# calmiLovesAI/ComputerVision.pytorch

Measured on AMD Instinct MI355X. Metric: images/sec 640x640 YOLOv8-n train step, higher is better.
Workload: dtype f16; 1 GPU; YOLOv8-n train step (fwd + v8 loss + bwd + Adam), batch 32/GPU, 640x640, nc=80, random init; global_batch=32, parallelism=dp1, launch=eager, exchange=none (1 rank), gpu_max_hw_queues=4

## Files before the change

computervision.pytorch_amd/csrc/stem.hip:

```cpp
#include "stem.h"

#include "bn_common.h"

namespace {
using namespace cvx_bn;

constexpr int KT = 27;

struct PixelId {
  int b, oy, ox;
};
__device__ __forceinline__ PixelId pixel_of(const StemParams& p, long long m) {
  const unsigned mu = (unsigned)m;
  const unsigned t = mu / (unsigned)p.OW;
  const int ox = (int)(mu - t * (unsigned)p.OW);
  const int b = (int)(t / (unsigned)p.OH);
  const int oy = (int)(t - (unsigned)b * (unsigned)p.OH);
  return PixelId{b, oy, ox};
}

__device__ __forceinline__ void load_window(const StemParams& p, const PixelId& id, float (&x)[KT]) {
  const long long plane = (long long)p.H * p.W;
  const float* img = p.img + (long long)id.b * 3 * plane;
#pragma unroll
  for (int kh = 0; kh < 3; ++kh) {
    const int iy = 2 * id.oy - 1 + kh;
    const bool rok = iy >= 0;
    const int iyc = rok ? iy : 0;
#pragma unroll
    for (int ci = 0; ci < 3; ++ci) {
      const float* row = img + ci * plane + (long long)iyc * p.W + 2 * id.ox;
      const float2 c = *reinterpret_cast<const float2*>(row);
      const float l = id.ox > 0 ? row[-1] : 0.f;
      x[(kh * 3 + 0) * 3 + ci] = rok ? l : 0.f;
      x[(kh * 3 + 1) * 3 + ci] = rok ? c.x : 0.f;
      x[(kh * 3 + 2) * 3 + ci] = rok ? c.y : 0.f;
    }
  }
}

__device__ __forceinline__ void stage_weights(const StemParams& p, float* sW) {
  for (int i = threadIdx.x; i < KT * p.Cout; i += blockDim.x) {
    const int co = i / KT, k = i - co * KT;
    sW[k * p.Cout + co] = p.w[i];
  }
}

__device__ __forceinline__ void conv16(const float (&x)[KT], const float* sW, int Cout, int g, float (&acc)[16]) {
#pragma unroll
  for (int c = 0; c < 16; ++c) acc[c] = 0.f;
#pragma unroll
  for (int k = 0; k < KT; ++k) {
    const f4* w4 = reinterpret_cast<const f4*>(sW + k * Cout + g * 16);
#pragma unroll
    for (int q = 0; q < 4; ++q) {
      const f4 w = w4[q];
#pragma unroll
      for (int r = 0; r < 4; ++r) acc[q * 4 + r] = fmaf(x[k], w[r], acc[q * 4 + r]);
    }
  }
}

template <int NG>
__global__ __launch_bounds__(256) void stem_stats_kernel(const StemParams p, long long M, long long* stats) {
  extern __shared__ __attribute__((aligned(16))) float smem[];
  float* sW = smem;
  float* sred = smem + KT * p.Cout;
  stage_weights(p, sW);
  __syncthreads();
  float s1[NG][16], s2[NG][16];
#pragma unroll
  for (int g = 0; g < NG; ++g)
#pragma unroll
    for (int c = 0; c < 16; ++c) s1[g][c] = s2[g][c] = 0.f;
  for (long long m = (long long)blockIdx.x * 256 + threadIdx.x; m < M; m += (long long)gridDim.x * 256) {
    asm volatile("" ::: "memory");
    const PixelId id = pixel_of(p, m);
    float x[KT];
    load_window(p, id, x);
#pragma unroll
    for (int g = 0; g < NG; ++g) {
      float acc[16];
      conv16(x, sW, p.Cout, g, acc);
#pragma unroll
      for (int c = 0; c < 16; ++c) {
        s1[g][c] += acc[c];
        s2[g][c] = fmaf(acc[c], acc[c], s2[g][c]);
      }
    }
  }
  const int wave = threadIdx.x >> 6, lane = threadIdx.x & 63;
#pragma unroll
  for (int g = 0; g < NG; ++g)
#pragma unroll
    for (int c = 0; c < 16; ++c) {
      const float a = cvx_wave_sum64(s1[g][c]), b = cvx_wave_sum64(s2[g][c]);
      if (lane == 0) {
        sred[(wave * 2 + 0) * p.Cout + g * 16 + c] = a;
        sred[(wave * 2 + 1) * p.Cout + g * 16 + c] = b;
      }
    }
  __syncthreads();
  for (int t = threadIdx.x; t < 2 * p.Cout; t += 256) {
    const int which = t / p.Cout, c = t - which * p.Cout;
    const float v = (sred[(0 * 2 + which) * p.Cout + c] + sred[(1 * 2 + which) * p.Cout + c]) +
                    (sred[(2 * 2 + which) * p.Cout + c] + sred[(3 * 2 + which) * p.Cout + c]);
    cvx_fix_atomic_add(stats, ((long long)(blockIdx.x % cvx_stat_replicas(p.Cout)) * p.Cout + c) * 2 + which, v);
  }
}

template <int NG, bool TRAIN>
__global__ __launch_bounds__(256) void stem_apply_kernel(const StemParams p, long long M, BnTrainArgs a, const float* scale,
                                                         const float* shift, ViewDesc out, half_t* xhat) {
  extern __shared__ __attribute__((aligned(16))) long long ws[];
  float* sA = reinterpret_cast<float*>(reinterpret_cast<char*>(ws) + (TRAIN ? fold_ws_bytes(p.Cout) : 0));
  float* sB = sA + p.Cout;
  float* sG = sB + p.Cout;
  float* sBe = sG + p.Cout;
  float* sW = sBe + p.Cout;
  if (TRAIN) {
    fold_replicas(a.stats, p.Cout, ws);
    for (int c = threadIdx.x; c < p.Cout; c += 256) {
      double var;
      const BnMoments mo = moments_of(ws, p.Cout, c, M, a.eps, &var);
      sA[c] = mo.mean;
      sB[c] = mo.invstd;
      sG[c] = a.gamma[c];
      sBe[c] = a.beta[c];
      if (blockIdx.x == 0) {
        const double cnt = (double)M;
        const double mu = reinterpret_cast<const double*>(ws)[c] / cnt;
        a.mean[c] = mo.mean;
        a.invstd[c] = mo.invstd;
        const double unbiased = cnt > 1.0 ? var * cnt / (cnt - 1.0) : var;
        a.rmean[c] = (float)((1.0 - a.momentum) * (double)a.rmean[c] + a.momentum * mu);
        a.rvar[c] = (float)((1.0 - a.momentum) * (double)a.rvar[c] + a.momentum * unbiased);
      }
    }
  } else {
    for (int c = threadIdx.x; c < p.Cout; c += 256) {
      sA[c] = scale[c];
      sB[c] = shift[c];
    }
  }
  stage_weights(p, sW);
  __syncthreads();
  const int ohw = p.OH * p.OW;
  for (long long m = (long long)blockIdx.x * 256 + threadIdx.x; m < M; m += (long long)gridDim.x * 256) {
    asm volatile("" ::: "memory");
    const PixelId id = pixel_of(p, m);
    float x[KT];
    load_window(p, id, x);
    half_t* o = out.p + (long long)id.b * out.bstride + ((long long)id.oy * p.OW + id.ox) * out.ld;
#pragma unroll
    for (int g = 0; g < NG; ++g) {
      float acc[16];
      conv16(x, sW, p.Cout, g, acc);
      h8 av[2], xv[2];
#pragma unroll
      for (int c = 0; c < 16; ++c) {
        const int ch = g * 16 + c;
        float z;
        if (TRAIN) {
          const float xh = (acc[c] - sA[ch]) * sB[ch];
          xv[c >> 3][c & 7] = (half_t)xh;
          z = fmaf(xh, sG[ch], sBe[ch]);
        } else {
          z = fmaf(acc[c], sA[ch], sB[ch]);
        }
        av[c >> 3][c & 7] = (half_t)cvx_silu(z);
      }
      *reinterpret_cast<h8*>(o + g * 16) = av[0];
      *reinterpret_cast<h8*>(o + g * 16 + 8) = av[1];
      if (TRAIN && xhat) {
        half_t* xo = xhat + m * p.Cout + g * 16;
        *reinterpret_cast<h8*>(xo) = xv[0];
        *reinterpret_cast<h8*>(xo + 8) = xv[1];
      }
    }
  }
  (void)ohw;
}

__global__ __launch_bounds__(256) void stem_wgrad_kernel(const StemParams p, long long M, const half_t* dy, float* slabs) {
  const int wave = threadIdx.x >> 6, lane = threadIdx.x & 63;
  const int co0 = blockIdx.y * 16 + wave * 4;
  float acc[4][KT];
#pragma unroll
  for (int c = 0; c < 4; ++c)
#pragma unroll
    for (int k = 0; k < KT; ++k) acc[c][k] = 0.f;
  constexpr int WG_UNR = 3;
  const long long stride = (long long)gridDim.x * 64;
  for (long long m0 = (long long)blockIdx.x * 64 + lane; m0 < M; m0 += stride * WG_UNR) {
    asm volatile("" ::: "memory");
    float x[WG_UNR][KT];
    h4 g[WG_UNR];
#pragma unroll
    for (int u = 0; u < WG_UNR; ++u) {
      const long long m = m0 + u * stride;
      const bool ok = m < M;
      const long long mm = ok ? m : m0;
      load_window(p, pixel_of(p, mm), x[u]);
      g[u] = *reinterpret_cast<const h4*>(dy + mm * p.Cout + co0);
      if (!ok) g[u] = h4{(half_t)0, (half_t)0, (half_t)0, (half_t)0};
    }
#pragma unroll
    for (int u = 0; u < WG_UNR; ++u)
#pragma unroll
      for (int c = 0; c < 4; ++c) {
        const float gc = (float)g[u][c];
#pragma unroll
        for (int k = 0; k < KT; ++k) acc[c][k] = fmaf(gc, x[u][k], acc[c][k]);
      }
  }
  float* slab = slabs + (long long)blockIdx.x * p.Cout * 144;
#pragma unroll
  for (int c = 0; c < 4; ++c)
#pragma unroll
    for (int k = 0; k < KT; ++k) {
      const float v = cvx_wave_sum64(acc[c][k]);
      if (lane == 0) slab[(co0 + c) * 144 + (k / 3) * 16 + (k % 3)] = v;
    }
}

__global__ __launch_bounds__(256) void stem_bwd_kernel(const StemParams p, long long M, const half_t* xhat, ViewDesc gout, BnCoef k,
                                                       const long long* part, float inv_scale, float* dgamma, float* dbeta, float* slabs,
                                                       int tiles_x, int tiles_y, int total_tiles) {
  constexpr int TH = 8, TW = 32, WR = 2 * TH + 1, WE = TW + 1, WO = TW;
  constexpr int ROWP = WE + WO + 1;
  extern __shared__ __attribute__((aligned(16))) long long ws[];
  float* sG = reinterpret_cast<float*>(reinterpret_cast<char*>(ws) + fold_ws_bytes(p.Cout));
  float* sB = sG + p.Cout;
  float* sK1 = sB + p.Cout;
  float* sK2 = sK1 + p.Cout;
  float* sGi = sK2 + p.Cout;
  float* sX = sGi + p.Cout;
  fold_replicas(part, p.Cout, ws);
  {
    const double* s0 = reinterpret_cast<const double*>(ws);
    const double* s1 = s0 + p.Cout;
    const double cnt = (double)M;
    for (int c = threadIdx.x; c < p.Cout; c += 256) {
      const float g = k.gamma[c];
      sG[c] = g;
      sB[c] = k.beta[c];
      sK1[c] = (float)(s0[c] / cnt);
      sK2[c] = (float)(s1[c] / cnt);
      sGi[c] = g * k.invstd[c];
      if (blockIdx.x == 0 && blockIdx.y == 0) {
        dgamma[c] += (float)(s1[c] * inv_scale);
        dbeta[c] += (float)(s0[c] * inv_scale);
      }
    }
  }
  __syncthreads();
  const int wave = threadIdx.x >> 6, lane = threadIdx.x & 63;
  const int co0 = blockIdx.y * 16 + wave * 4;
  float ga[4], be[4], k1[4], k2[4], gi[4];
#pragma unroll
  for (int c = 0; c < 4; ++c) {
    ga[c] = sG[co0 + c];
    be[c] = sB[co0 + c];
    k1[c] = sK1[co0 + c];
    k2[c] = sK2[co0 + c];
    gi[c] = sGi[co0 + c];
  }
  float acc[4][KT];
#pragma unroll
  for (int c = 0; c < 4; ++c)
#pragma unroll
    for (int kk = 0; kk < KT; ++kk) acc[c][kk] = 0.f;
  const long long plane = (long long)p.H * p.W;
  const int lx = lane & 31, ly = lane >> 5;
  for (int tile = blockIdx.x; tile < total_tiles; tile += gridDim.x) {
    const int tx = tile % tiles_x;
    const int t2 = tile / tiles_x;
    const int ty = t2 % tiles_y;
    const int b = t2 / tiles_y;
    const int oy0 = ty * TH, ox0 = tx * TW;
    auto load_group = [&](int q, h4& xq, h4& gq, bool& okq) {
      const int oy = oy0 + q * 2 + ly, ox = ox0 + lx;
      okq = oy < p.OH && ox < p.OW;
      const long long pix = okq ? (long long)oy * p.OW + ox : 0;
      xq = *reinterpret_cast<const h4*>(xhat + ((long long)b * p.OH * p.OW + pix) * p.Cout + co0);
      gq = *reinterpret_cast<const h4*>(gout.p + (long long)b * gout.bstride + pix * gout.ld + co0);
    };
    h4 xn, gn;
    bool okn;
    load_group(0, xn, gn, okn);
    const float* img = p.img + (long long)b * 3 * plane;
    __syncthreads();
    {
      constexpr int NE = 3 * WR * (WE + WO), NST = (NE + 255) / 256;
      float v[NST];
      int dst[NST];
#pragma unroll
      for (int it = 0; it < NST; ++it) {
        const int e = it * 256 + threadIdx.x;
        const int j = e % (WE + WO);
        const int t3 = e / (WE + WO);
        const int r = t3 % WR, ci = t3 / WR;
        const int iy = 2 * oy0 - 1 + r, ix = 2 * ox0 - 1 + j;
        const bool in = e < NE && iy >= 0 && iy < p.H && ix >= 0 && ix < p.W;
        v[it] = in ? img[ci * plane + (long long)iy * p.W + ix] : 0.f;
        dst[it] = e < NE ? (ci * WR + r) * ROWP + ((j & 1) ? WE + (j >> 1) : (j >> 1)) : -1;
      }
#pragma unroll
      for (int it = 0; it < NST; ++it)
        if (dst[it] >= 0) sX[dst[it]] = v[it];
    }
    __syncthreads();
#pragma unroll 1
    for (int q = 0; q < 4; ++q) {
      const h4 xq = xn, gq = gn;
      const bool okq = okn;
      if (q < 3) load_group(q + 1, xn, gn, okn);
      float dyc[4];
#pragma unroll
      for (int c = 0; c < 4; ++c) {
        const float xv = (float)xq[c];
        const float dz = (float)gq[c] * cvx_silu_grad(xv * ga[c] + be[c]);
        dyc[c] = okq ? (float)(half_t)(gi[c] * (dz - k1[c] - xv * k2[c])) : 0.f;
      }
      const float* rowq = sX + (2 * (q * 2 + ly)) * ROWP;
#pragma unroll
      for (int kh = 0; kh < 3; ++kh)
#pragma unroll
        for (int ci = 0; ci < 3; ++ci) {
          const float* row = rowq + (ci * WR + kh) * ROWP;
          const float x0 = row[lx], x1 = row[WE + lx], x2 = row[lx + 1];
#pragma unroll
          for (int c = 0; c < 4; ++c) {
            acc[c][(kh * 3 + 0) * 3 + ci] = fmaf(dyc[c], x0, acc[c][(kh * 3 + 0) * 3 + ci]);
            acc[c][(kh * 3 + 1) * 3 + ci] = fmaf(dyc[c], x1, acc[c][(kh * 3 + 1) * 3 + ci]);
            acc[c][(kh * 3 + 2) * 3 + ci] = fmaf(dyc[c], x2, acc[c][(kh * 3 + 2) * 3 + ci]);
          }
        }
    }
  }
  float* slab = slabs + (long long)blockIdx.x * p.Cout * 144;
#pragma unroll
  for (int c = 0; c < 4; ++c)
#pragma unroll
    for (int kk = 0; kk < KT; ++kk) {
      const float v = cvx_wave_sum64(acc[c][kk]);
      if (lane == 0) slab[(co0 + c) * 144 + (kk / 3) * 16 + (kk % 3)] = v;
    }
}

constexpr int SM_TH = 8, SM_TW = 32, SM_WR = 2 * SM_TH + 1, SM_P = 72, SM_PL = SM_WR * SM_P + 16;
constexpr int SM_WIN_CHUNKS = 16 * 64;
constexpr int SM_STAGE_BYTES = SM_WIN_CHUNKS * 16 + 2 * SM_TH * SM_TW * 32;
static_assert(3 * SM_PL / 4 <= SM_WIN_CHUNKS, "window chunks");

typedef __attribute__((address_space(3))) void* stem_lds_ptr;

constexpr int SM_PART = 16 * 32 * 2 + 32 + 16 + 16;

template <bool ONEPASS, bool RECOMP = false>
__global__ __launch_bounds__(256) void stem_bwd_mfma_kernel(const StemParams p, long long M, const half_t* xhat, ViewDesc gout, BnCoef k,
                                                            const long long* part, float inv_scale, float* dgamma, float* dbeta, float* slabs,
                                                            int tiles_x, int tiles_y, int total_tiles) {
#if defined(__HIP_DEVICE_COMPILE__)
  extern __shared__ __attribute__((aligned(16))) long long ws[];
  float* sG = reinterpret_cast<float*>(reinterpret_cast<char*>(ws) + fold_ws_bytes(p.Cout));
  float* sB = sG + p.Cout;
  float* sK1 = sB + p.Cout;
  float* sK2 = sK1 + p.Cout;
  float* sGi = sK2 + p.Cout;
  unsigned char* stage0 = reinterpret_cast<unsigned char*>(reinterpret_cast<uintptr_t>(sGi + p.Cout + 3) & ~(uintptr_t)15);
  const int wave = __builtin_amdgcn_readfirstlane(threadIdx.x >> 6), lane = threadIdx.x & 63;
  const int g = lane >> 4, m = lane & 15;
  const int co0 = blockIdx.y * 16;
  const long long plane = (long long)p.H * p.W;

  const __amdgpu_buffer_rsrc_t rs_img = __builtin_amdgcn_make_buffer_rsrc(const_cast<float*>(p.img), (short)0, (int)(unsigned)((long long)p.B * 3 * plane * 4), 0x00020000);
  const __amdgpu_buffer_rsrc_t rs_xh = __builtin_amdgcn_make_buffer_rsrc(const_cast<half_t*>(xhat), (short)0, (int)(unsigned)(M * p.Cout * 2), 0x00020000);
  const __amdgpu_buffer_rsrc_t rs_g = __builtin_amdgcn_make_buffer_rsrc(gout.p, (short)0, (int)(unsigned)((long long)p.B * gout.bstride * 2), 0x00020000);

  int w_rel[4], w_r[4], w_j[4];
#pragma unroll
  for (int j = 0; j < 4; ++j) {
    const int chunk = (4 * j + wave) * 64 + lane;
    const int ci = chunk / (SM_PL / 4), rem = chunk - ci * (SM_PL / 4);
    const int r = rem / (SM_P / 4), cj = rem - r * (SM_P / 4);
    const bool used = ci < 3 && r < SM_WR && cj < 17;
    w_r[j] = used ? r : -100000;
    w_j[j] = cj;
    w_rel[j] = (int)((ci * (long long)p.H + (r - 1)) * p.W + (4 * cj - 4)) * 4;
  }
  const int t_px = lane >> 1, t_half = lane & 1;

  auto issue = [&](int tile, unsigned char* st) {
    const int tx = tile % tiles_x;
    const int t2 = tile / tiles_x;
    const int ty = t2 % tiles_y;
    const int b = t2 / tiles_y;
    const int oy0 = ty * SM_TH, ox0 = tx * SM_TW;
    const unsigned base = (unsigned)((((long long)b * 3 * p.H + 2 * oy0) * p.W + 2 * ox0) * 4);
#pragma unroll
    for (int j = 0; j < 4; ++j) {
      const int iy = 2 * oy0 - 1 + w_r[j], ix = 2 * ox0 - 4 + 4 * w_j[j];
      const bool ok = iy >= 0 && iy < p.H && ix >= 0 && ix < p.W;
      const unsigned vo = ok ? base + (unsigned)w_rel[j] : 0xffffffffu;
      __builtin_amdgcn_raw_ptr_buffer_load_lds(rs_img, (stem_lds_ptr)(st + (4 * j + wave) * 1024), 16, vo, 0, 0, 0);
    }
    unsigned char* sx = st + SM_WIN_CHUNKS * 16;
    unsigned char* sg = sx + (RECOMP ? 0 : SM_TH * SM_TW * 32);
#pragma unroll
    for (int j = 0; j < 2; ++j) {
      const int row = 2 * wave + j;
      const int oy = oy0 + row, ox = ox0 + t_px;
      const bool ok = oy < p.OH && ox < p.OW;
      const long long pix = (long long)oy * p.OW + ox;
      const unsigned vx = ok ? (unsigned)((((long long)b * p.OH * p.OW + pix) * p.Cout + co0) * 2 + t_half * 16) : 0xffffffffu;
      const unsigned vg = ok ? (unsigned)(((long long)b * gout.bstride + pix * gout.ld + co0) * 2 + t_half * 16) : 0xffffffffu;
      if constexpr (!RECOMP) __builtin_amdgcn_raw_ptr_buffer_load_lds(rs_xh, (stem_lds_ptr)(sx + row * 1024), 16, vx, 0, 0, 0);
      __builtin_amdgcn_raw_ptr_buffer_load_lds(rs_g, (stem_lds_ptr)(sg + row * 1024), 16, vg, 0, 0, 0);
    }
  };

  int tile = blockIdx.x;
  if (tile < total_tiles) issue(tile, stage0);

  float k1 = 0.f, k2 = 0.f, gi = 0.f;
  if constexpr (!ONEPASS) {
    fold_replicas(part, p.Cout, ws);
    const double* s0 = reinterpret_cast<const double*>(ws);
    const double* s1 = s0 + p.Cout;
    const double cnt = (double)M;
    for (int c = threadIdx.x; c < p.Cout; c += 256) {
      const float gm = k.gamma[c];
      sK1[c] = (float)(s0[c] / cnt);
      sK2[c] = (float)(s1[c] / cnt);
      sGi[c] = gm * k.invstd[c];
      if (blockIdx.x == 0 && blockIdx.y == 0) {
        dgamma[c] += (float)(s1[c] * inv_scale);
        dbeta[c] += (float)(s0[c] * inv_scale);
      }
    }
    __syncthreads();
    k1 = sK1[co0 + m];
    k2 = sK2[co0 + m];
    gi = sGi[co0 + m];
  }
  const float ga = k.gamma[co0 + m], be = k.beta[co0 + m];

  int boff[2];
#pragma unroll
  for (int t = 0; t < 2; ++t) {
    const int kk = min(16 * t + m, KT - 1);
    const int ci = kk % 3, kw = (kk / 3) % 3, kh = kk / 9;
    boff[t] = (ci * SM_PL + (4 * wave + kh) * SM_P + kw + 3 + 2 * g) * 4;
  }
  const int aoff = (2 * wave * SM_TW + g) * 32 + m * 2;
  int toff7[7], boffr[2];
  float wreg[7];
  float mean_c = 0.f, invstd_c = 0.f;
  if constexpr (RECOMP) {
#pragma unroll
    for (int t = 0; t < 7; ++t) {
      const int kq = 4 * t + g, kk = min(kq, KT - 1);
      const int ci = kk % 3, kw = (kk / 3) % 3, kh = kk / 9;
      toff7[t] = (ci * SM_PL + (4 * wave + kh) * SM_P + kw + 3 + 2 * m) * 4;
      wreg[t] = kq < KT ? p.w[(long long)(co0 + m) * KT + kq] : 0.f;
    }
#pragma unroll
    for (int t = 0; t < 2; ++t) boffr[t] = boff[t] + (2 * (4 * g) - 2 * g) * 4;
    mean_c = k.mean[co0 + m];
    invstd_c = k.invstd[co0 + m];
  }
  const int aoffr = (2 * wave * SM_TW + 4 * g) * 32 + m * 2;

  f4 acc0 = {0.f, 0.f, 0.f, 0.f}, acc1 = {0.f, 0.f, 0.f, 0.f};
  f4 acx0 = {0.f, 0.f, 0.f, 0.f}, acx1 = {0.f, 0.f, 0.f, 0.f};
  float sdz = 0.f, sdzx = 0.f, sb0 = 0.f, sb1 = 0.f;
  int cur = 0;
  for (; tile < total_tiles; tile += gridDim.x) {
    constexpr int STAGE = SM_STAGE_BYTES - (RECOMP ? SM_TH * SM_TW * 32 : 0);
    unsigned char* st = stage0 + cur * STAGE;
    asm volatile("s_waitcnt vmcnt(0)" ::: "memory");
    asm volatile("" ::: "memory");
    __builtin_amdgcn_s_barrier();
    asm volatile("" ::: "memory");
    if (tile + (int)gridDim.x < total_tiles) issue(tile + gridDim.x, stage0 + (cur ^ 1) * STAGE);
    const int tx = tile % tiles_x, ty = (tile / tiles_x) % tiles_y;
    const int oy0 = ty * SM_TH + 2 * wave, ox0 = tx * SM_TW + g;
    const unsigned char* sw = st;
    const unsigned char* sx = st + SM_WIN_CHUNKS * 16 + aoff;
    const unsigned char* sg = sx + SM_TH * SM_TW * 32;
    if constexpr (ONEPASS && RECOMP) {
      const unsigned char* sgr = st + SM_WIN_CHUNKS * 16 + aoffr;
      const int oxb = tx * SM_TW + 4 * g;
#pragma unroll
      for (int q = 0; q < 4; ++q) {
        const int row = q >> 1, cb = (q & 1) * 16;
        f4 y = {0.f, 0.f, 0.f, 0.f};
#pragma unroll
        for (int t = 0; t < 7; ++t) {
          const float a = *reinterpret_cast<const float*>(sw + toff7[t] + (row * 2 * SM_P + 2 * cb) * 4);
          y = __builtin_amdgcn_mfma_f32_16x16x4f32(a, wreg[t], y, 0, 0, 0);
        }
        typedef _Float16 hv4 __attribute__((ext_vector_type(4)));
        hv4 dz4, xv4, b04, b14;
#pragma unroll
        for (int i = 0; i < 4; ++i) {
          const bool ok = oy0 + row < p.OH && oxb + cb + i < p.OW;
          const half_t xh = (half_t)((y[i] - mean_c) * invstd_c);
          const float xv = ok ? (float)xh : 0.f;
          const float gv = (float)*reinterpret_cast<const half_t*>(sgr + (row * SM_TW + cb + i) * 32);
          const half_t b0 = (half_t)*reinterpret_cast<const float*>(sw + boffr[0] + (row * 2 * SM_P + 2 * (cb + i)) * 4);
          const half_t b1 = (half_t)*reinterpret_cast<const float*>(sw + boffr[1] + (row * 2 * SM_P + 2 * (cb + i)) * 4);
          const half_t dzh = (half_t)(gv * cvx_silu_grad(xv * ga + be));
          const float dz = (float)dzh;
          dz4[i] = dzh;
          xv4[i] = (half_t)xv;
          b04[i] = b0;
          b14[i] = b1;
          sdz += dz;
          sdzx = fmaf(dz, xv, sdzx);
          sb0 += ok ? (float)b0 : 0.f;
          sb1 += ok ? (float)b1 : 0.f;
        }
        acc0 = __builtin_amdgcn_mfma_f32_16x16x16f16(dz4, b04, acc0, 0, 0, 0);
        acc1 = __builtin_amdgcn_mfma_f32_16x16x16f16(dz4, b14, acc1, 0, 0, 0);
        acx0 = __builtin_amdgcn_mfma_f32_16x16x16f16(xv4, b04, acx0, 0, 0, 0);
        acx1 = __builtin_amdgcn_mfma_f32_16x16x16f16(xv4, b14, acx1, 0, 0, 0);
      }
    } else {
#pragma unroll
    for (int s = 0; s < 16; ++s) {
      const int row = s >> 3, c4 = (s & 7) * 4;
      const float xv = (float)*reinterpret_cast<const half_t*>(sx + s * 128);
      const float gv = (float)*reinterpret_cast<const half_t*>(sg + s * 128);
      const float b0 = *reinterpret_cast<const float*>(sw + boff[0] + (row * 2 * SM_P + 2 * c4) * 4);
      const float b1 = *reinterpret_cast<const float*>(sw + boff[1] + (row * 2 * SM_P + 2 * c4) * 4);
      const bool ok = oy0 + row < p.OH && ox0 + c4 < p.OW;
      const float dz = gv * cvx_silu_grad(xv * ga + be);
      if constexpr (ONEPASS) {
        acc0 = __builtin_amdgcn_mfma_f32_16x16x4f32(dz, b0, acc0, 0, 0, 0);
        acc1 = __builtin_amdgcn_mfma_f32_16x16x4f32(dz, b1, acc1, 0, 0, 0);
        acx0 = __builtin_amdgcn_mfma_f32_16x16x4f32(xv, b0, acx0, 0, 0, 0);
        acx1 = __builtin_amdgcn_mfma_f32_16x16x4f32(xv, b1, acx1, 0, 0, 0);
        sdz += dz;
        sdzx = fmaf(dz, xv, sdzx);
        sb0 += ok ? b0 : 0.f;
        sb1 += ok ? b1 : 0.f;
      } else {
        const float dy = ok ? (float)(half_t)(gi * (dz - k1 - xv * k2)) : 0.f;
        acc0 = __builtin_amdgcn_mfma_f32_16x16x4f32(dy, b0, acc0, 0, 0, 0);
        acc1 = __builtin_amdgcn_mfma_f32_16x16x4f32(dy, b1, acc1, 0, 0, 0);
      }
    }
    }
    cur ^= 1;
  }
  if constexpr (ONEPASS) {
    __syncthreads();
    float* red = reinterpret_cast<float*>(stage0);
    float* mine = red + wave * SM_PART;
    sdz += __shfl_xor(sdz, 16);
    sdz += __shfl_xor(sdz, 32);
    sdzx += __shfl_xor(sdzx, 16);
    sdzx += __shfl_xor(sdzx, 32);
    sb0 += __shfl_xor(sb0, 16);
    sb0 += __shfl_xor(sb0, 32);
    sb1 += __shfl_xor(sb1, 16);
    sb1 += __shfl_xor(sb1, 32);
#pragma unroll
    for (int i = 0; i < 4; ++i) {
      mine[(4 * g + i) * 32 + m] = acc0[i];
      mine[(4 * g + i) * 32 + 16 + m] = acc1[i];
      mine[512 + (4 * g + i) * 32 + m] = acx0[i];
      mine[512 + (4 * g + i) * 32 + 16 + m] = acx1[i];
    }
    if (g == 0) {
      mine[1024 + m] = sb0;
      mine[1024 + 16 + m] = sb1;
      mine[1056 + m] = sdz;
      mine[1072 + m] = sdzx;
    }
    __syncthreads();
    float* out = slabs + (long long)blockIdx.x * p.Cout * 144 + blockIdx.y * (16 * 144);
    for (int e = threadIdx.x; e < SM_PART; e += 256) out[e] = ((red[e] + red[e + SM_PART]) + red[e + 2 * SM_PART]) + red[e + 3 * SM_PART];
    if (blockIdx.x == 0 && threadIdx.x == 0) reinterpret_cast<unsigned*>(out)[2 * SM_PART + 64] = 0u;
    return;
  }
  __syncthreads();
  float* red = reinterpret_cast<float*>(stage0);
#pragma unroll
  for (int i = 0; i < 4; ++i) {
    red[((wave * 2 + 0) * 4 + i) * 64 + lane] = acc0[i];
    red[((wave * 2 + 1) * 4 + i) * 64 + lane] = acc1[i];
  }
  __syncthreads();
  float* slab = slabs + (long long)blockIdx.x * p.Cout * 144;
  for (int e = threadIdx.x; e < 512; e += 256) {
    const int l = e & 63, i = (e >> 6) & 3, t = e >> 8;
    const int kk = 16 * t + (l & 15), co = 4 * (l >> 4) + i;
    if (kk < KT) {
      const int q = (t * 4 + i) * 64 + l;
      const float v = ((red[q] + red[q + 512]) + red[q + 1024]) + red[q + 1536];
      slab[(co0 + co) * 144 + (kk / 3) * 16 + (kk % 3)] = v;
    }
  }
#endif
}

constexpr int SM_FOLD_BLOCKS = SM_PART / 16;
__global__ __launch_bounds__(256) void stem_onepass_fold_kernel(float* slabs, int nsplit, int Cout, long long M, const float* gamma, const float* invstd,
                                                                float inv_scale, float* dw, float* dgamma, float* dbeta) {
  __shared__ double sd[256];
  __shared__ double col[SM_PART];
  __shared__ bool last;
  const int slice = blockIdx.y;
  const long long stride = (long long)Cout * 144;
  float* base = slabs + slice * (16 * 144);
  const int c = threadIdx.x & 15, r = threadIdx.x >> 4;
  const int column = blockIdx.x * 16 + c;
  double a = 0.0;
  int sp = r;
  for (; sp + 7 * 16 < nsplit; sp += 8 * 16) {
    float v[8];
#pragma unroll
    for (int u = 0; u < 8; ++u) v[u] = base[(long long)(sp + 16 * u) * stride + column];
#pragma unroll
    for (int u = 0; u < 8; ++u) a += (double)v[u];
  }
  for (; sp < nsplit; sp += 16) a += (double)base[(long long)sp * stride + column];
  sd[threadIdx.x] = a;
  __syncthreads();
  for (int off = 128; off >= 16; off >>= 1) {
    if ((int)threadIdx.x < off) sd[threadIdx.x] += sd[threadIdx.x + off];
    __syncthreads();
  }
  auto colsum_at = [&](int q) -> double* { return reinterpret_cast<double*>(base + (long long)(q / 544) * stride + SM_PART) + (q % 544); };
  if (threadIdx.x < 16) __hip_atomic_store(colsum_at(column), sd[threadIdx.x], __ATOMIC_RELAXED, __HIP_MEMORY_SCOPE_AGENT);
  __syncthreads();
  if (threadIdx.x == 0) {
    __threadfence();
    unsigned* ctr = reinterpret_cast<unsigned*>(base) + 2 * SM_PART + 64;
    last = atomicAdd(ctr, 1u) == gridDim.x - 1;
    if (last) __threadfence();
  }
  __syncthreads();
  if (!last) return;
  for (int q = threadIdx.x; q < SM_PART; q += 256) col[q] = __hip_atomic_load(colsum_at(q), __ATOMIC_RELAXED, __HIP_MEMORY_SCOPE_AGENT);
  __syncthreads();
  const double cnt = (double)M;
  for (int e = threadIdx.x; e < 16 * KT; e += 256) {
    const int co = e / KT, kk = e - co * KT;
    const double k1 = col[1056 + co] / cnt, k2 = col[1072 + co] / cnt;
    const double g = (double)gamma[slice * 16 + co] * (double)invstd[slice * 16 + co];
    const double v = g * (col[co * 32 + kk] - k1 * col[1024 + kk] - k2 * col[512 + co * 32 + kk]);
    dw[(long long)(slice * 16 + co) * KT + kk] += (float)(v * inv_scale);
  }
  if (threadIdx.x < 16) {
    dgamma[slice * 16 + threadIdx.x] += (float)(col[1072 + threadIdx.x] * inv_scale);
    dbeta[slice * 16 + threadIdx.x] += (float)(col[1056 + threadIdx.x] * inv_scale);
  }
}

__global__ __launch_bounds__(256) void stem_slab_fold_kernel(const float* slabs, int nsplit, int Cout, float inv_scale, float* dw) {
  const int e = blockIdx.x * 256 + threadIdx.x;
  if (e >= Cout * KT) return;
  const int co = e / KT, kk = e - co * KT;
  const float* s = slabs + (long long)co * 144 + (kk / 3) * 16 + (kk % 3);
  float a = 0.f;
  for (int sp = 0; sp < nsplit; ++sp) a += s[(long long)sp * Cout * 144];
  dw[e] += a * inv_scale;
}

int stem_grid(long long M, int per_block) {
  long long blocks = (M + per_block - 1) / per_block;
  const long long cap = 256 * 8;
  return (int)(blocks < cap ? blocks : cap);
}

int check(const StemParams& p) {
  CVX_CHECK(p.img && p.w, "stem: null pointers");
  CVX_CHECK(p.H % 2 == 0 && p.W % 2 == 0 && p.OH == p.H / 2 && p.OW == p.W / 2, "stem: even input sizes, output = input / 2");
  CVX_CHECK(p.Cout % 16 == 0 && p.Cout >= 16 && p.Cout <= 80, "stem: 16..80 output channels in multiples of 16");
  CVX_CHECK((long long)p.B * p.OH * p.OW < (1LL << 31), "stem: too many output pixels");
  CVX_CHECK(((uintptr_t)p.img % 8) == 0, "stem: images must be 8-byte aligned");
  return 0;
}

}

int cvx_stem_stats(const StemParams& p, long long* stats, hipStream_t st) {
  CVX_TRY(check(p));
  const long long M = (long long)p.B * p.OH * p.OW;
  const int lds = (KT + 8) * p.Cout * 4;
  const dim3 grid(stem_grid(M, 256));
  switch (p.Cout / 16) {
    case 1: hipLaunchKernelGGL(stem_stats_kernel<1>, grid, dim3(256), lds, st, p, M, stats); break;
    case 2: hipLaunchKernelGGL(stem_stats_kernel<2>, grid, dim3(256), lds, st, p, M, stats); break;
    case 3: hipLaunchKernelGGL(stem_stats_kernel<3>, grid, dim3(256), lds, st, p, M, stats); break;
    case 4: hipLaunchKernelGGL(stem_stats_kernel<4>, grid, dim3(256), lds, st, p, M, stats); break;
    default: hipLaunchKernelGGL(stem_stats_kernel<5>, grid, dim3(256), lds, st, p, M, stats); break;
  }
  CVX_HIP(hipGetLastError());
  return 0;
}

template <bool TRAIN>
static int launch_apply(const StemParams& p, const BnTrainArgs& a, const float* scale, const float* shift, const ViewDesc& out,
                        half_t* xhat, hipStream_t st) {
  const long long M = (long long)p.B * p.OH * p.OW;
  const int lds = (TRAIN ? fold_ws_bytes(p.Cout) : 0) + (4 + KT) * p.Cout * 4;
  const dim3 grid(stem_grid(M, 256));
  switch (p.Cout / 16) {
    case 1: hipLaunchKernelGGL((stem_apply_kernel<1, TRAIN>), grid, dim3(256), lds, st, p, M, a, scale, shift, out, xhat); break;
    case 2: hipLaunchKernelGGL((stem_apply_kernel<2, TRAIN>), grid, dim3(256), lds, st, p, M, a, scale, shift, out, xhat); break;
    case 3: hipLaunchKernelGGL((stem_apply_kernel<3, TRAIN>), grid, dim3(256), lds, st, p, M, a, scale, shift, out, xhat); break;
    case 4: hipLaunchKernelGGL((stem_apply_kernel<4, TRAIN>), grid, dim3(256), lds, st, p, M, a, scale, shift, out, xhat); break;
    default: hipLaunchKernelGGL((stem_apply_kernel<5, TRAIN>), grid, dim3(256), lds, st, p, M, a, scale, shift, out, xhat); break;
  }
  CVX_HIP(hipGetLastError());
  return 0;
}

int cvx_stem_apply_train(const StemParams& p, const BnTrainArgs& a, const ViewDesc& out, half_t* xhat, hipStream_t st) {
  CVX_TRY(check(p));
  CVX_CHECK(out.p && ((uintptr_t)out.p % 16) == 0 && out.ld % 8 == 0, "stem: output view");
  return launch_apply<true>(p, a, nullptr, nullptr, out, xhat, st);
}

int cvx_stem_apply_eval(const StemParams& p, const float* scale, const float* shift, const ViewDesc& out, hipStream_t st) {
  CVX_TRY(check(p));
  CVX_CHECK(out.p && scale && shift && ((uintptr_t)out.p % 16) == 0 && out.ld % 8 == 0, "stem: output view");
  BnTrainArgs none{};
  return launch_apply<false>(p, none, scale, shift, out, nullptr, st);
}

int cvx_stem_wgrad_splits(long long M) {
  static const int cap = cvx_tune_int("CVX_STEM_SPLITS", 512);
  return stem_grid(M, 64 * 16) < cap ? stem_grid(M, 64 * 16) : cap;
}

int cvx_stem_wgrad(const StemParams& p, const half_t* dy, float* slabs, int nsplit, hipStream_t st) {
  CVX_TRY(check(p));
  const long long M = (long long)p.B * p.OH * p.OW;
  CVX_CHECK(dy && slabs && nsplit >= 1 && nsplit == cvx_stem_wgrad_splits(M), "stem wgrad: split count must come from cvx_stem_wgrad_splits");
  hipLaunchKernelGGL(stem_wgrad_kernel, dim3(nsplit, p.Cout / 16), dim3(256), 0, st, p, M, dy, slabs);
  CVX_HIP(hipGetLastError());
  return 0;
}

int cvx_stem_backward(const StemParams& p, const half_t* xhat, const ViewDesc& gout, const BnCoef& k, const long long* part, float inv_scale,
                      float* dgamma, float* dbeta, float* slabs, int nsplit, hipStream_t st) {
  CVX_TRY(check(p));
  const long long M = (long long)p.B * p.OH * p.OW;
  CVX_CHECK(xhat && gout.p && part && dgamma && dbeta && slabs && nsplit == cvx_stem_wgrad_splits(M), "stem backward: bad arguments");
  CVX_CHECK(gout.ld % 4 == 0 && ((uintptr_t)gout.p % 8) == 0, "stem backward: gradient view alignment");
  const int tiles_x = (p.OW + 31) / 32, tiles_y = (p.OH + 7) / 8;
  static const bool mfma_on = cvx_tune_int("CVX_STEM_BWD_MFMA", 1) != 0;
  const bool mfma_ok = mfma_on && p.W % 4 == 0 && ((uintptr_t)p.img % 16) == 0 && ((uintptr_t)xhat % 16) == 0 && ((uintptr_t)gout.p % 16) == 0 &&
                       gout.ld % 8 == 0 && gout.bstride % 8 == 0 && (long long)p.B * 3 * p.H * p.W * 4 < (1LL << 32) && M * p.Cout * 2 < (1LL << 32) &&
                       (long long)p.B * gout.bstride * 2 < (1LL << 32);
  if (mfma_ok) {
    const int lds_m = fold_ws_bytes(p.Cout) + 5 * p.Cout * 4 + 32 + 2 * SM_STAGE_BYTES;
    hipLaunchKernelGGL(stem_bwd_mfma_kernel<false>, dim3(nsplit, p.Cout / 16), dim3(256), lds_m, st, p, M, xhat, gout, k, part, inv_scale, dgamma, dbeta,
                       slabs, tiles_x, tiles_y, tiles_x * tiles_y * p.B);
    CVX_HIP(hipGetLastError());
    return 0;
  }
  const int lds = fold_ws_bytes(p.Cout) + 5 * p.Cout * 4 + 3 * 17 * 66 * 4;
  hipLaunchKernelGGL(stem_bwd_kernel, dim3(nsplit, p.Cout / 16), dim3(256), lds, st, p, M, xhat, gout, k, part, inv_scale, dgamma, dbeta, slabs,
                     tiles_x, tiles_y, tiles_x * tiles_y * p.B);
  CVX_HIP(hipGetLastError());
  return 0;
}

static bool stem_dma_ok(const StemParams& p, const half_t* xhat, const ViewDesc& gout, long long M) {
  return p.W % 4 == 0 && ((uintptr_t)p.img % 16) == 0 && ((uintptr_t)xhat % 16) == 0 && ((uintptr_t)gout.p % 16) == 0 && gout.ld % 8 == 0 &&
         gout.bstride % 8 == 0 && (long long)p.B * 3 * p.H * p.W * 4 < (1LL << 32) && M * p.Cout * 2 < (1LL << 32) &&
         (long long)p.B * gout.bstride * 2 < (1LL << 32);
}
bool cvx_stem_keeps_xhat(const StemParams& p, const ViewDesc& gout, int nsplit) {
  static const bool recomp = cvx_tune_int("CVX_STEM_RECOMP", 1) != 0;
  return !(recomp && cvx_stem_backward_onepass_ok(p, reinterpret_cast<const half_t*>((uintptr_t)16), gout, nsplit));
}
bool cvx_stem_backward_onepass_ok(const StemParams& p, const half_t* xhat, const ViewDesc& gout, int nsplit) {
  static const bool on = cvx_tune_int("CVX_STEM_ONEPASS", 1) != 0;
  const long long M = (long long)p.B * p.OH * p.OW;
  return on && nsplit >= 2 && p.Cout % 16 == 0 && stem_dma_ok(p, xhat, gout, M);
}
int cvx_stem_backward_fold(const StemParams& p, const half_t* xhat, const ViewDesc& gout, const BnCoef& k, const long long* part, float inv_scale,
                           float* dgamma, float* dbeta, float* dw, float* slabs, int nsplit, hipStream_t st) {
  CVX_TRY(check(p));
  const long long M = (long long)p.B * p.OH * p.OW;
  CVX_CHECK(xhat && gout.p && dgamma && dbeta && dw && slabs && nsplit == cvx_stem_wgrad_splits(M), "stem backward: bad arguments");
  if (cvx_stem_backward_onepass_ok(p, xhat, gout, nsplit)) {
    const int tiles_x = (p.OW + 31) / 32, tiles_y = (p.OH + 7) / 8;
    const int lds_m = fold_ws_bytes(p.Cout) + 5 * p.Cout * 4 + 32 + 2 * SM_STAGE_BYTES;
    if (k.mean && !cvx_stem_keeps_xhat(p, gout, nsplit)) {
      hipLaunchKernelGGL((stem_bwd_mfma_kernel<true, true>), dim3(nsplit, p.Cout / 16), dim3(256), lds_m - 2 * SM_TH * SM_TW * 32, st, p, M, xhat, gout, k, (const long long*)nullptr,
                         inv_scale, dgamma, dbeta, slabs, tiles_x, tiles_y, tiles_x * tiles_y * p.B);
    } else
    hipLaunchKernelGGL(stem_bwd_mfma_kernel<true>, dim3(nsplit, p.Cout / 16), dim3(256), lds_m, st, p, M, xhat, gout, k, (const long long*)nullptr, inv_scale,
                       dgamma, dbeta, slabs, tiles_x, tiles_y, tiles_x * tiles_y * p.B);
    hipLaunchKernelGGL(stem_onepass_fold_kernel, dim3(SM_FOLD_BLOCKS, p.Cout / 16), dim3(256), 0, st, slabs, nsplit, p.Cout, M, k.gamma, k.invstd, inv_scale,
                       dw, dgamma, dbeta);
    CVX_HIP(hipGetLastError());
    return 0;
  }
  CVX_CHECK(part, "stem backward: the two-pass path needs the sums of bn_bwd_reduce");
  CVX_TRY(cvx_stem_backward(p, xhat, gout, k, part, inv_scale, dgamma, dbeta, slabs, nsplit, st));
  hipLaunchKernelGGL(stem_slab_fold_kernel, dim3((p.Cout * KT + 255) / 256), dim3(256), 0, st, slabs, nsplit, p.Cout, inv_scale, dw);
  CVX_HIP(hipGetLastError());
  return 0;
}
```

Measured before the change: 5676 images/sec.

## Add quad-tiled stem stats kernel that shares input windows across 2x2 outputs

```diff
diff --git a/computervision.pytorch_amd/csrc/stem.hip b/computervision.pytorch_amd/csrc/stem.hip
--- a/computervision.pytorch_amd/csrc/stem.hip
+++ b/computervision.pytorch_amd/csrc/stem.hip
@@ -180,6 +180,152 @@
     }
   }
   (void)ohw;
+}
+
+struct QuadId {
+  int b, rp, cp;
+};
+__device__ __forceinline__ QuadId quad_of(int q, int RP, int CP) {
+  const unsigned t = (unsigned)q / (unsigned)CP;
+  const int cp = (int)((unsigned)q - t * (unsigned)CP);
+  const int b = (int)(t / (unsigned)RP);
+  return QuadId{b, (int)(t - (unsigned)b * (unsigned)RP), cp};
+}
+constexpr int QW = 5 * 3;
+
+__device__ __forceinline__ void load_quad(const StemParams& p, const QuadId& id, int lane, f4 (&c)[QW], float (&l)[QW]) {
+  const long long plane = (long long)p.H * p.W;
+  const float* img = p.img + (long long)id.b * 3 * plane + 4 * id.cp;
+  const float* row[QW];
+#pragma unroll
+  for (int r = 0; r < 5; ++r) {
+    const int iy = 4 * id.rp - 1 + r;
+    const int iyc = iy < 0 ? 0 : (iy < p.H ? iy : p.H - 1);
+#pragma unroll
+    for (int ci = 0; ci < 3; ++ci) {
+      row[r * 3 + ci] = img + ci * plane + (long long)iyc * p.W;
+      c[r * 3 + ci] = *reinterpret_cast<const f4*>(row[r * 3 + ci]);
+      l[r * 3 + ci] = 0.f;
+    }
+  }
+  if (lane == 0 && id.cp > 0) {
+#pragma unroll
+    for (int i = 0; i < QW; ++i) l[i] = row[i][-1];
+  }
+}
+__device__ __forceinline__ void build_window(const QuadId& id, int lane, bool bot, const f4 (&c)[QW], const float (&l)[QW], float (&x)[5 * QW]) {
+  const bool from_lane = lane != 0 && id.cp > 0;
+#pragma unroll
+  for (int r = 0; r < 5; ++r) {
+    const bool rok = r == 0 ? id.rp > 0 : (r >= 3 ? bot : true);
+#pragma unroll
+    for (int ci = 0; ci < 3; ++ci) {
+      const f4 v = c[r * 3 + ci];
+      const float prev = cvx_dpp_mov<0x138>(v[3]);
+      x[(r * 5 + 0) * 3 + ci] = rok ? (from_lane ? prev : l[r * 3 + ci]) : 0.f;
+#pragma unroll
+      for (int j = 0; j < 4; ++j) x[(r * 5 + 1 + j) * 3 + ci] = rok ? v[j] : 0.f;
+    }
+  }
+}
+__device__ __forceinline__ void conv16_quad(const float (&x)[5 * QW], const float* sW, int Cout, int g, f4 (&acc)[4][4]) {
+#pragma unroll
+  for (int px = 0; px < 4; ++px)
+#pragma unroll
+    for (int q = 0; q < 4; ++q) acc[px][q] = f4{0.f, 0.f, 0.f, 0.f};
+  const f4* w4 = reinterpret_cast<const f4*>(sW + g * 16);
+  f4 wn[4];
+#pragma unroll
+  for (int q = 0; q < 4; ++q) wn[q] = w4[q];
+#pragma unroll
+  for (int k = 0; k < KT; ++k) {
+    const int kh = k / 9, kw = (k / 3) % 3, ci = k % 3;
+    f4 wk[4];
+#pragma unroll
+    for (int q = 0; q < 4; ++q) wk[q] = wn[q];
+    if (k + 1 < KT) {
+#pragma unroll
+      for (int q = 0; q < 4; ++q) wn[q] = w4[(k + 1) * (Cout / 4) + q];
+    }
+    asm volatile("" : "+v"(wk[0]), "+v"(wk[1]), "+v"(wk[2]), "+v"(wk[3]) : : "memory");
+#pragma unroll
+    for (int px = 0; px < 4; ++px) asm volatile("" : "+v"(acc[px][0]), "+v"(acc[px][1]), "+v"(acc[px][2]), "+v"(acc[px][3]));
+#pragma unroll
+    for (int q = 0; q < 4; ++q) {
+#pragma unroll
+      for (int px = 0; px < 4; ++px) {
+        const float xv = x[((2 * (px >> 1) + kh) * 5 + 2 * (px & 1) + kw) * 3 + ci];
+#pragma unroll
+        for (int r = 0; r < 4; ++r) acc[px][q][r] = fmaf(xv, wk[q][r], acc[px][q][r]);
+      }
+    }
+  }
+}
+__device__ __forceinline__ void quad_range(int Q, int& begin, int& end) {
+  const long long tiles = ((long long)Q + 255) / 256;
+  begin = (int)(tiles * blockIdx.x / gridDim.x) * 256;
+  const long long e = tiles * (blockIdx.x + 1) / gridDim.x * 256;
+  end = (int)(e < Q ? e : Q);
+}
+
+template <int NG>
+__global__ __launch_bounds__(256) void stem_stats_tile_kernel(const StemParams p, int RP, int CP, int Q, long long* stats) {
+  extern __shared__ __attribute__((aligned(16))) float smem[];
+  float* sW = smem;
+  float* sred = smem + KT * p.Cout;
+  stage_weights(p, sW);
+  __syncthreads();
+  float s1[NG][16], s2[NG][16];
+#pragma unroll
+  for (int g = 0; g < NG; ++g)
+#pragma unroll
+    for (int c = 0; c < 16; ++c) s1[g][c] = s2[g][c] = 0.f;
+  const int wave = threadIdx.x >> 6, lane = threadIdx.x & 63;
+  int begin, end;
+  quad_range(Q, begin, end);
+  int qw = begin + wave * 64;
+  for (; qw < end; qw += 256) {
+    asm volatile("" ::: "memory");
+    const bool ok = qw + lane < end;
+    const QuadId id = quad_of(min(qw + lane, end - 1), RP, CP);
+    const bool bot = 4 * id.rp + 2 < p.H;
+    f4 rc[QW];
+    float rl[QW], x[5 * QW];
+    load_quad(p, id, lane, rc, rl);
+    build_window(id, lane, bot, rc, rl, x);
+    const bool ok1 = ok && bot;
+#pragma unroll
+    for (int g = 0; g < NG; ++g) {
+      f4 acc[4][4];
+      conv16_quad(x, sW, p.Cout, g, acc);
+#pragma unroll
+      for (int c = 0; c < 16; ++c) {
+#pragma unroll
+        for (int px = 0; px < 4; ++px) {
+          const float v = (px < 2 ? ok : ok1) ? acc[px][c >> 2][c & 3] : 0.f;
+          s1[g][c] += v;
+          s2[g][c] = fmaf(v, v, s2[g][c]);
+        }
+      }
+    }
+  }
+#pragma unroll
+  for (int g = 0; g < NG; ++g)
+#pragma unroll
+    for (int c = 0; c < 16; ++c) {
+      const float a = cvx_wave_sum64(s1[g][c]), b = cvx_wave_sum64(s2[g][c]);
+      if (lane == 0) {
+        sred[(wave * 2 + 0) * p.Cout + g * 16 + c] = a;
+        sred[(wave * 2 + 1) * p.Cout + g * 16 + c] = b;
+      }
+    }
+  __syncthreads();
+  for (int t = threadIdx.x; t < 2 * p.Cout; t += 256) {
+    const int which = t / p.Cout, c = t - which * p.Cout;
+    const float v = (sred[(0 * 2 + which) * p.Cout + c] + sred[(1 * 2 + which) * p.Cout + c]) +
+                    (sred[(2 * 2 + which) * p.Cout + c] + sred[(3 * 2 + which) * p.Cout + c]);
+    cvx_fix_atomic_add(stats, ((long long)(blockIdx.x % cvx_stat_replicas(p.Cout)) * p.Cout + c) * 2 + which, v);
+  }
 }
 
 __global__ __launch_bounds__(256) void stem_wgrad_kernel(const StemParams p, long long M, const half_t* dy, float* slabs) {
@@ -687,12 +833,43 @@
   return 0;
 }
 
+struct QuadGeom {
+  int RP, CP, Q, grid;
+};
+bool quad_ok(const StemParams& p) {
+  static const bool on = cvx_tune_int("CVX_STEM_TILE", 1) != 0;
+  return on && p.W % 4 == 0 && ((uintptr_t)p.img % 16) == 0;
+}
+QuadGeom quad_geom(const StemParams& p) {
+  QuadGeom q;
+  q.RP = (p.OH + 1) / 2;
+  q.CP = p.OW / 2;
+  q.Q = p.B * q.RP * q.CP;
+  const int cap = p.Cout == 16 ? 512 : 256;
+  const int tiles = (q.Q + 255) / 256;
+  q.grid = tiles < cap ? tiles : cap;
+  return q;
+}
+
 }
 
 int cvx_stem_stats(const StemParams& p, long long* stats, hipStream_t st) {
   CVX_TRY(check(p));
   const long long M = (long long)p.B * p.OH * p.OW;
   const int lds = (KT + 8) * p.Cout * 4;
+  if (quad_ok(p)) {
+    const QuadGeom q = quad_geom(p);
+    const dim3 qgrid(q.grid);
+    switch (p.Cout / 16) {
+      case 1: hipLaunchKernelGGL(stem_stats_tile_kernel<1>, qgrid, dim3(256), lds, st, p, q.RP, q.CP, q.Q, stats); break;
+      case 2: hipLaunchKernelGGL(stem_stats_tile_kernel<2>, qgrid, dim3(256), lds, st, p, q.RP, q.CP, q.Q, stats); break;
+      case 3: hipLaunchKernelGGL(stem_stats_tile_kernel<3>, qgrid, dim3(256), lds, st, p, q.RP, q.CP, q.Q, stats); break;
+      case 4: hipLaunchKernelGGL(stem_stats_tile_kernel<4>, qgrid, dim3(256), lds, st, p, q.RP, q.CP, q.Q, stats); break;
+      default: hipLaunchKernelGGL(stem_stats_tile_kernel<5>, qgrid, dim3(256), lds, st, p, q.RP, q.CP, q.Q, stats); break;
+    }
+    CVX_HIP(hipGetLastError());
+    return 0;
+  }
   const dim3 grid(stem_grid(M, 256));
   switch (p.Cout / 16) {
     case 1: hipLaunchKernelGGL(stem_stats_kernel<1>, grid, dim3(256), lds, st, p, M, stats); break;
```

New measurement: 5636 images/sec. Within noise of the previous version (-0.7%).
